# gorse-io/gorse

Hardware: AMD Instinct MI355X
Metric: BPR positive-samples/sec (whole job, N GPUs) (higher is better)
Workload: dtype f32; 1 GPU; S-ml1m 6040x3706x994169 per rank (C2), nFactors=64; factors_finite=True

## Files before the change

### gorse_amd/capi.py

```python
import ctypes as C
import os

import numpy as np

HERE = os.path.dirname(os.path.abspath(__file__))
LIB_PATH = os.environ.get("GORSE_HIP_LIB") or os.path.join(HERE, "lib", "libgorse_hip.so")

OK, ERR_INVALID, ERR_HIP, ERR_CANCELLED, ERR_NO_DEVICE, ERR_RANGE, ERR_NOMEM = 0, -1, -2, -3, -4, -5, -6
BPR_HOGWILD_ATOMIC, BPR_SEQUENTIAL, BPR_HOGWILD_RACY, BPR_HOGWILD_STORES = 0, 1, 2, 3
DTYPE_F32, DTYPE_BF16 = 0, 1
METRIC_NEG_DOT, METRIC_EUCLIDEAN, METRIC_COSINE, METRIC_EUCLIDEAN_BF16 = 0, 1, 2, 3
PROF_BPR_UPDATE, PROF_BPR_SAMPLE, PROF_ALS_SWEEP, PROF_ALS_GRAM, PROF_BPR_SORT, PROF_COMM = 0, 1, 2, 3, 4, 5
COMM_ID_BYTES = 128
OPT_SGD, OPT_ADAM = 0, 1
PROF_TOPK_SCORE, PROF_TOPK_RESCORE, PROF_TOPK_SWEEP, PROF_TOPK_SELECT, PROF_TOPK_HIST, PROF_TOPK_REPLAY = 0, 1, 2, 3, 4, 5

_f32p = C.POINTER(C.c_float)
_i32p = C.POINTER(C.c_int32)
_i64p = C.POINTER(C.c_int64)
_f64p = C.POINTER(C.c_double)
_vp = C.c_void_p

SIGNATURES = {
    "gorse_hip_abi_version": (C.c_int32, []),
# ... 115 lines not shown
    "gorse_hip_test_set_sparse_table": (None, [C.c_int32]),
    "gorse_hip_test_set_sparse_probe": (None, [C.c_int32]),
    "gorse_hip_test_set_sparse_sym": (None, [C.c_int32, C.c_int32, C.c_int32, C.c_int32]),
    "gorse_hip_test_set_sparse_front": (None, [C.c_int32]),
    "gorse_hip_test_sparse_sym_stats": (None, [C.c_void_p, C.POINTER(C.c_int64)]),
    "gorse_hip_test_set_sparse_tile": (None, [C.c_int32]),
    "gorse_hip_test_set_scan_literal": (None, [C.c_int32]),
    "gorse_hip_test_set_stream_priorities": (None, [C.c_int32]),
    "gorse_hip_test_set_sparse_split": (None, [C.c_int64]),
    "gorse_hip_test_set_sparse_heavy": (None, [C.c_int64]),
    "gorse_hip_test_set_sparse_atomic": (None, [C.c_int32]),
    "gorse_hip_test_set_als_path": (None, [C.c_int32]),
    "gorse_hip_test_set_als_plan": (None, [C.c_int32, C.c_int32]),
    "gorse_hip_test_set_bpr_chunk": (None, [C.c_int64]),
    "gorse_hip_test_bpr_prepare_chunk": (C.c_int32, [_vp, C.c_int64, C.c_uint64, C.c_uint64, C.c_int64, _i32p, _i32p, _i32p]),
    "gorse_hip_test_bpr_finish_capacities": (None, [_i32p, _i32p]),
    "gorse_hip_test_bpr_fail_count": (C.c_int32, [_vp, _i32p]),
    "gorse_hip_test_set_bpr_store_mode": (None, [C.c_int32]),
    "gorse_hip_test_set_prep_cu_stride": (None, [C.c_int32]),
    "gorse_hip_test_set_sgemm_valu": (None, [C.c_int32]),
    "gorse_hip_test_sgemm_last_ms": (C.c_double, []),
    "gorse_hip_test_set_bpr_cold_window": (None, [C.c_int64]),
    "gorse_hip_test_set_bpr_replica_unit": (None, [C.c_double]),
    "gorse_hip_test_set_bpr_fold_period": (None, [C.c_int32]),
    "gorse_hip_test_bpr_fold_stats": (C.c_int32, [_vp, _vp]),
    "gorse_hip_test_bpr_hot_state": (C.c_int32, [_vp, _vp, _vp, _vp]),
    "gorse_hip_test_set_recommend": (None, [C.c_int32, C.c_int32, C.c_int64]),
    "gorse_hip_test_set_fm_rank": (None, [C.c_int64, C.c_int32]),
    "gorse_hip_test_fm_rank_sort": (C.c_int32, [_vp, C.c_int64, _i64p, _f32p, _i32p]),
    "gorse_hip_test_set_fm_evaluate": (None, [C.c_int64, C.c_int32]),
# ... 161 lines not shown
    def bpr_sample_triplets(self, n, seed, epoch, sample_base=0):
        u = np.empty(n, np.int32)
        i = np.empty(n, np.int32)
        j = np.empty(n, np.int32)
        check(lib().gorse_bpr_sample_triplets(self.h, n, seed, epoch, sample_base, _p(u, _i32p), _p(i, _i32p),
                                              _p(j, _i32p)))
        return u, i, j

    def bpr_prepare_chunk(self, n, seed, epoch, sample_base=0):
        off = np.empty(self.U + 2, np.int32)
        si = np.empty(n, np.int32)
        sj = np.empty(n, np.int32)
        check(lib().gorse_hip_test_bpr_prepare_chunk(self.h, n, seed, epoch, sample_base, _p(off, _i32p), _p(si, _i32p),
                                                     _p(sj, _i32p)))
        return off, si, sj

    def bpr_fail_count(self):
        n = C.c_int32(0)
        check(lib().gorse_hip_test_bpr_fail_count(self.h, C.byref(n)))
        return n.value

    def bpr_apply_triplets(self, u, i, j, lr, reg, mode):
        u, i, j = _arr(u, np.int32), _arr(i, np.int32), _arr(j, np.int32)
        if not (u.size == i.size == j.size):
            raise GorseHipError(ERR_INVALID, "triplet arrays differ in length")
        check(lib().gorse_bpr_apply_triplets(self.h, _p(u, _i32p), _p(i, _i32p), _p(j, _i32p), u.size, lr, reg, mode))

    def als_epoch(self, weight, reg, cancel=None):
        cp = _p(cancel, _i32p) if cancel is not None else None
        check(lib().gorse_als_epoch(self.h, weight, reg, cp))
# ... 625 lines not shown
```

### gorse_amd/csrc/bpr.hip

```cpp
#include <algorithm>
#include <cstdlib>
#include <cstring>

#include "bpr_bins.hpp"
#include "mf_internal.hpp"
#include <utility>

using namespace gorse;

namespace {

int g_variant = 0;
constexpr int MODE_ATOMIC = GORSE_BPR_HOGWILD_ATOMIC;
constexpr int MODE_EXACT = GORSE_BPR_SEQUENTIAL;
constexpr int MODE_RACY = GORSE_BPR_HOGWILD_RACY;
constexpr int MODE_STORES = GORSE_BPR_HOGWILD_STORES;

__device__ __forceinline__ bool row_contains(const int32_t *__restrict__ row, int64_t n, int32_t x) {
    int64_t lo = 0, hi = n;
    while (lo < hi) {
        int64_t mid = (lo + hi) >> 1;
        if (row[mid] < x)
            lo = mid + 1;
        else
// ... 977 lines not shown
        su[pos] = us[s];
        si[pos] = is[s];
        sj[pos] = js[s];
    }
}

constexpr int kCold = -2;
constexpr int kSeriesFlush = 8;
#ifndef GORSE_BPR_SERIES_SKIP_GATHERS
#define GORSE_BPR_SERIES_SKIP_GATHERS 1
#endif

#ifndef GORSE_BPR_D8_PAIRS
#define GORSE_BPR_D8_PAIRS 1
#endif
template <int NC, bool NEG_STORE, bool D8 = false>
__global__ __launch_bounds__(kBlock) void bpr_update_user_kernel(float *P, float *Q, const int32_t *__restrict__ si,
                                                                 const int32_t *__restrict__ sj,
                                                                 const int32_t *__restrict__ off, int32_t U, int d,
                                                                 float lr, float reg, int exp_mode, double *loss,
                                                                 HotRows hot, int folders, int neg_replicas) {
    if ((int)blockIdx.x < folders) {
        run_folders<true>(hot, Q, folders);
        return;
    }
    auto continues = [](int i0, int j0, int i1, int j1) { return i0 == i1 && (i0 | j0 | j1) >= 0 && i0 != j0 && i0 != j1; };
    const int glane = threadIdx.x & (kGroup - 1);
    const int lane = D8 ? (glane & 7) : glane;
    constexpr int SUBS = D8 && GORSE_BPR_D8_PAIRS ? 2 : 1;
    const bool writer = !D8 || SUBS == 2 || glane < 8;
    auto mad = [](float x, float y, float z) { return D8 ? x * y + z : fmaf(x, y, z); };
    auto tree8 = [](float v) { return SUBS == 2 ? group_tree8_halves(v) : group_tree8(v); };
    const int gib = threadIdx.x / kGroup;
    const int64_t group = ((int64_t)((int)blockIdx.x - folders) * kGroupsPerBlock + gib) * SUBS + (SUBS == 2 ? glane >> 3 : 0);
    const int64_t ngroups = (int64_t)((int)gridDim.x - folders) * kGroupsPerBlock * SUBS;
    const float nreg = -reg;
    double my_loss = 0.0;
    const bool look_i = hot.n_hot > 0;
    const bool look_j = (hot.n_hot > 0 && neg_replicas) || NEG_STORE;
    const int32_t *slot_of = (look_i || look_j) ? hot.slot : si;
    int im1 = -1, jm1 = -1, im2 = -1, jm2 = -1;
    for (int64_t u = group; u < U; u += ngroups) {
        const int beg = off[u], end = off[u + 1];
        if (beg >= end) continue;
        float *pu = P + u * d;
        constexpr int G = 2, IA = 3;
        constexpr int GB = NEG_STORE ? 1 : G;
        float p[NC], ra[G][NC], rb[GB][NC];
        const int last = end - 1;
        auto at = [&](int s) { return s <= last ? s : last; };
// ... 137 lines not shown
int32_t exclusive_scan_i32(int32_t *data, int64_t m, int32_t *tmp, hipStream_t st) {
    const int64_t nt = ceil_div(m, kScanTile);
    if (nt <= 16) {
        scan_small_kernel<<<dim3(1), dim3(256), 0, st>>>(data, m);
        GORSE_HIP_CHECK(hipGetLastError());
        return GORSE_OK;
    }
    scan_tile_sums_kernel<<<dim3((unsigned)nt), dim3(256), 0, st>>>(data, m, tmp);
    scan_sums_kernel<<<dim3(1), dim3(256), 0, st>>>(tmp, nt);
    scan_apply_kernel<<<dim3((unsigned)nt), dim3(256), 0, st>>>(data, m, tmp);
    GORSE_HIP_CHECK(hipGetLastError());
    return GORSE_OK;
}


int32_t launch_user_sort(gorse_mf *h, const int32_t *trip, int32_t *sorted, int32_t *bucket, int32_t *rank, int64_t n, size_t cap,
                         hipStream_t st, bool ranked) {
    const int64_t m = h->U + 2;
    const int64_t blocks = std::min<int64_t>(ceil_div(n, 256), 256 * 8);
    if (!ranked) {
        GORSE_HIP_CHECK(hipMemsetAsync(bucket, 0, (size_t)m * sizeof(int32_t), st));
        if (g_variant & (1 << 29))
            bpr_rank_kernel<<<dim3(1), dim3(1), 0, st>>>(trip, n, (int32_t)h->U, bucket, rank);
        else
            bpr_rank_kernel<<<dim3((unsigned)blocks), dim3(256), 0, st>>>(trip, n, (int32_t)h->U, bucket, rank);
    }
    GORSE_TRY(exclusive_scan_i32(bucket, m, h->scan_tmp2.p, st));
    bpr_scatter_by_kernel<<<dim3((unsigned)blocks), dim3(256), 0, st>>>(trip, trip, trip + cap, trip + 2 * cap, n,
                                                                       (int32_t)h->U, bucket, rank, sorted,
                                                                       sorted + cap, sorted + 2 * cap);
    GORSE_HIP_CHECK(hipGetLastError());
    return GORSE_OK;
}
int32_t ensure_user_sort(gorse_mf *h) {
    const int64_t m = h->U + 2;
    const size_t mat = prep_matrix_words(h->U, (int64_t)h->trip_cap);
    if ((size_t)m <= h->ubucket[0].n && h->scan_tmp2.n >= (size_t)ceil_div(m, kScanTile) && h->urank[0].n >= 2 * h->trip_cap &&
        h->ubins.n >= (size_t)2 * kMaxBins && h->ubinmat.n >= mat)
        return GORSE_OK;
    GORSE_TRY(mf_sync_streams(h));
    if (h->ubins.n < (size_t)2 * kMaxBins) GORSE_TRY(h->ubins.alloc((size_t)2 * kMaxBins));
    if (h->ubinmat.n < mat) GORSE_TRY(h->ubinmat.alloc(mat));
    for (int b = 0; b < 2; b++) {
        GORSE_TRY(h->ubucket[b].alloc((size_t)m));
        GORSE_TRY(h->urank[b].alloc(2 * h->trip_cap));
    }
    if (h->scan_tmp2.n < (size_t)ceil_div(m, kScanTile)) GORSE_TRY(h->scan_tmp2.alloc((size_t)ceil_div(m, kScanTile)));
    return GORSE_OK;
}
bool user_runs_supported(const gorse_mf *h) {
    return (h->d == 8 || h->d == 16 || h->d == 32 || h->d == 64 || h->d == 128) && (h->U >= 4096 || (g_variant & 128));
}

constexpr int kDefaultStoreMode = 1;
int g_store_mode = kDefaultStoreMode;

HotRows make_hot(const gorse_mf *h) {
    return HotRows{h->hot_slot.p, h->hot_items.p, h->hot_meta.p, h->hot_rep.p, h->hot_done.p, 0, h->d, 0, g_fold_period};
}
int open_hot(gorse_mf *h, HotRows &hot) {
    hot.n_hot = h->n_hot;
    hot.set = (int)(h->hot_launches++ & 1);
    return kFolderBlocks;
}

int32_t launch_update_users(gorse_mf *h, const int32_t *sorted, const int32_t *bucket, size_t cap, float lr, float reg,
                            int exp_mode, double *loss, hipStream_t st, bool stores, hipEvent_t start = nullptr,
                            hipEvent_t stop = nullptr) {
    const int d = h->d;
    int64_t blocks = ceil_div(h->U, (int64_t)kGroupsPerBlock * (d == 8 && GORSE_BPR_D8_PAIRS ? 2 : 1));
    const int64_t capb = 256 * 16;
    if (blocks > capb) blocks = capb;
    HotRows hot = make_hot(h);
    const int folders = h->n_hot > 0 && !(g_variant & 32) ? open_hot(h, hot) : 0;
    blocks += folders;
    const int neg_rep = !(g_variant & (1 << 25)) && hot.n_hot > 0 && hot_neg_replicas(hot.n_hot, h->I) ? 1 : 0;
    dim3 grid((unsigned)blocks), block(kBlock);
    const bool neg_store = stores && h->n_cold > 0 && g_store_mode == 1;
#define LAUNCH2(NC, NEG_STORE)                                                                                         \
    hipExtLaunchKernelGGL((bpr_update_user_kernel<(NC == 0 ? 1 : NC), NEG_STORE, NC == 0>), grid, block, 0, st, start, stop, 0,     \
                          h->P.p, h->Q.p, sorted + cap, sorted + 2 * cap, bucket, (int32_t)h->U, d, lr, reg, exp_mode, loss, hot, \
                          folders, neg_rep)
#define LAUNCH(NC)                                                                                                     \
    do {                                                                                                               \
        if (neg_store)                                                                                                 \
            LAUNCH2(NC, true);                                                                                         \
        else                                                                                                           \
            LAUNCH2(NC, false);                                                                                        \
    } while (0)
    if (d == 8)
        LAUNCH(0);
    else if (d == 16)
        LAUNCH(1);
    else if (d == 32)
        LAUNCH(2);
    else if (d == 64)
        LAUNCH(4);
// ... 59 lines not shown
int32_t launch_sampler(gorse_mf *h, uint64_t seed, uint64_t epoch, int64_t base, int64_t n, int32_t *trip, size_t cap,
                       hipStream_t st, int32_t *bucket = nullptr, int32_t *rank = nullptr, hipEvent_t start = nullptr,
                       hipEvent_t stop = nullptr) {
    if (n <= 0) return GORSE_OK;
    int64_t blocks = std::min<int64_t>(ceil_div(n, 256), 256 * 8);
    if (bucket) GORSE_HIP_CHECK(hipMemsetAsync(bucket, 0, (size_t)(h->U + 2) * sizeof(int32_t), st));
    hipExtLaunchKernelGGL(bpr_sample_kernel, dim3((unsigned)blocks), dim3(256), 0, st, start, stop, 0, (int32_t)h->U, (int32_t)h->I,
                          h->uptr.p, h->uidx.p, h->uidx_sorted.p, seed, epoch, base, n, trip, trip + cap, trip + 2 * cap,
                          h->fail_count.p, bucket, rank);
    GORSE_HIP_CHECK(hipGetLastError());
    return GORSE_OK;
}

constexpr size_t kItemsBatchFrom = (size_t)8 << 20;
int32_t launch_prepare_users(gorse_mf *h, uint64_t seed, uint64_t epoch, int64_t base, int64_t n, int32_t *trip, int32_t *sorted,
                             int32_t *bucket, int32_t *rank, size_t cap, hipStream_t st) {
    if (n <= 0) return GORSE_OK;
    const int64_t m = h->U + 2;
    const int64_t blocks = std::min<int64_t>(ceil_div(n, 256), 256 * 8);
    const PrepBins pb = prep_bins(h->U, n);
    hipEvent_t ev_a = nullptr, ev_b = nullptr;
    auto launch_items = [&](const int2 *pairs) {
        h->prof.events(GORSE_PROF_BPR_SAMPLE, &ev_a, &ev_b);
        if (h->uidx.n > kItemsBatchFrom)
            hipExtLaunchKernelGGL(bpr_sample_items_batch_kernel, dim3((unsigned)blocks), dim3(256), 0, st, ev_a, ev_b, 0, (int32_t)h->U,
                                  (int32_t)h->I, h->uptr.p, h->uidx.p, h->uidx_sorted.p, seed, epoch, base, n, pairs, sorted + cap,
                                  sorted + 2 * cap, h->fail_count.p);
        else
            hipExtLaunchKernelGGL(bpr_sample_items_kernel, dim3((unsigned)blocks), dim3(256), 0, st, ev_a, ev_b, 0, (int32_t)h->U,
                                  (int32_t)h->I, h->uptr.p, h->uidx.p, h->uidx_sorted.p, seed, epoch, base, n, pairs, sorted + cap,
                                  sorted + 2 * cap, h->fail_count.p);
    };
    auto launch_group = [&]() {
        if (g_variant & (1 << 20)) return;
        h->prof.events(GORSE_PROF_BPR_SORT, &ev_a, &ev_b);
        hipExtLaunchKernelGGL(bpr_group_positives_kernel, dim3((unsigned)std::min<int64_t>(h->U, 256 * 16)), dim3(64), 0, st, ev_a, ev_b, 0,
                              (int32_t)h->U, bucket, sorted + cap, sorted + 2 * cap);
    };
    if (pb.ok && !(g_variant & (1 << 21))) {
        int32_t *key = trip;
        int2 *bp = reinterpret_cast<int2 *>(trip + cap), *pairs = reinterpret_cast<int2 *>(rank);
        int32_t *bin_count = h->ubins.p, *bin_start = h->ubins.p + kMaxBins, *H = h->ubinmat.p;
        const unsigned tiles = (unsigned)ceil_div(n, pb.tile);
        if ((size_t)tiles * pb.nbins > h->ubinmat.n) return fail(GORSE_ERR_INVALID, "tile x bin matrix smaller than %u x %d", tiles, pb.nbins);
        const bool finish = !(g_variant & (1 << 19)) && pb.shift <= kFinShift && n / pb.nbins <= kFinCap / 4 * 3 &&
                            h->uidx.n <= kItemsBatchFrom;
        h->prof.events(GORSE_PROF_BPR_SAMPLE, &ev_a, &ev_b);
        hipExtLaunchKernelGGL(bpr_bin_count_kernel, dim3(tiles), dim3(kBinThreads), 0, st, ev_a, ev_b, 0, (int32_t)h->U, h->uptr.p, seed,
                              epoch, base, n, pb.tile, pb.shift, pb.nbins, key, h->fail_count.p, H);
        h->prof.events(GORSE_PROF_BPR_SORT, &ev_a, &ev_b);
        hipExtLaunchKernelGGL(bpr_bin_offsets_kernel, dim3((unsigned)ceil_div(pb.nbins, 64)), dim3(kOffWaves * 64), 0, st, ev_a, nullptr, 0,
                              H, (int)tiles, pb.nbins, bin_count);
        hipExtLaunchKernelGGL(bpr_bin_scatter_kernel, dim3(tiles), dim3(kBinThreads), 0, st, nullptr, finish ? ev_b : nullptr, 0,
                              (int32_t)h->U, key, n, pb.tile, pb.shift, pb.nbins, bin_count, H, bin_start, bp);
        if (finish) {
            h->prof.events(GORSE_PROF_BPR_SAMPLE, &ev_a, &ev_b);
            hipExtLaunchKernelGGL(bpr_bin_finish_kernel, dim3((unsigned)pb.nbins), dim3(kFinThreads), 0, st, ev_a, ev_b, 0, (int32_t)h->U,
                                  (int32_t)h->I, pb.shift, bin_start, bp, h->uptr.p, h->uidx.p, h->uidx_sorted.p, seed, epoch, base, bucket,
                                  pairs, sorted + cap, sorted + 2 * cap, h->fail_count.p, (g_variant & (1 << 20)) ? 0 : 1);
            GORSE_HIP_CHECK(hipGetLastError());
            return GORSE_OK;
        }
        hipExtLaunchKernelGGL(bpr_bin_sort_kernel, dim3((unsigned)pb.nbins), dim3(256), 0, st, nullptr, ev_b, 0, (int32_t)h->U, pb.shift,
                              pb.nbins, bin_start, bp, bucket, pairs);
        launch_items(pairs);
        launch_group();
        GORSE_HIP_CHECK(hipGetLastError());
        return GORSE_OK;
    }
    int32_t *key = trip;
    int2 *pairs = reinterpret_cast<int2 *>(trip + cap);
    int tok = h->prof.begin(GORSE_PROF_BPR_SAMPLE, st);
    GORSE_HIP_CHECK(hipMemsetAsync(bucket, 0, (size_t)m * sizeof(int32_t), st));
    bpr_sample_user_kernel<<<dim3((unsigned)blocks), dim3(256), 0, st>>>((int32_t)h->U, h->uptr.p, seed, epoch, base, n, key,
                                                                         h->fail_count.p, bucket, rank);
    h->prof.end(tok, st);
    tok = h->prof.begin(GORSE_PROF_BPR_SORT, st);
    GORSE_TRY(exclusive_scan_i32(bucket, m, h->scan_tmp2.p, st));
    bpr_scatter_ids_kernel<<<dim3((unsigned)blocks), dim3(256), 0, st>>>(key, rank, bucket, n, (int32_t)h->U, pairs);
    h->prof.end(tok, st);
    launch_items(pairs);
    launch_group();
    GORSE_HIP_CHECK(hipGetLastError());
    return GORSE_OK;
}

int64_t g_chunk_override = 0;
int64_t chunk_capacity(const gorse_mf *h) {
    if (g_chunk_override > 0) return g_chunk_override;
    const int64_t lo = (int64_t)1 << 22, hi = (int64_t)1 << 27;
    return std::min(std::max(lo, 32 * h->U), hi);
}

int32_t ensure_trip(gorse_mf *h, int64_t want) {
    size_t cap = (size_t)std::min<int64_t>(std::max<int64_t>(want, 1), chunk_capacity(h));
    cap = (cap + 1) & ~(size_t)1;
    if (cap <= h->trip_cap) return GORSE_OK;
    GORSE_TRY(mf_sync_streams(h));
    for (int b = 0; b < 2; b++) GORSE_TRY(h->trip[b].alloc(cap * 3));
// ... 97 lines not shown
        if (uruns) GORSE_TRY(ensure_user_sort(h));
        int64_t c = 0;
        for (int64_t s0 = 0; s0 < n_samples; s0 += cap, c++) {
            const int b = (int)(h->chunk_seq & 1);
            h->chunk_seq++;
            const int64_t m = std::min(cap, n_samples - s0);
            if (cancel && *cancel) {
                GORSE_TRY(mf_sync_streams(h));
                return fail(GORSE_ERR_CANCELLED, "cancelled");
            }
            int32_t *tb = h->trip[b].p;
            const hipStream_t prep = (g_variant & (1 << 22)) ? h->stream : h->stream2;
            if (h->ev_consumed[b]) GORSE_HIP_CHECK(hipStreamWaitEvent(prep, h->ev_consumed[b], 0));
            const bool fused = uruns && !(g_variant & (1 << 29)) && !(g_variant & (1 << 27));
            const bool by_run = fused && !(g_variant & (1 << 26));
            if (by_run) {
                GORSE_TRY(launch_prepare_users(h, seed, epoch, base + s0, m, tb, h->sorted[b].p, h->ubucket[b].p, h->urank[b].p,
                                               (size_t)cap, prep));
            } else {
                int tok = fused ? h->prof.begin(GORSE_PROF_BPR_SAMPLE, prep) : -1;
                hipEvent_t sa = nullptr, sb = nullptr;
                if (!fused) h->prof.events(GORSE_PROF_BPR_SAMPLE, &sa, &sb);
                GORSE_TRY(launch_sampler(h, seed, epoch, base + s0, m, tb, (size_t)cap, prep, fused ? h->ubucket[b].p : nullptr,
                                         fused ? h->urank[b].p : nullptr, sa, sb));
                h->prof.end(tok, prep);
                if (fused) {
                    tok = h->prof.begin(GORSE_PROF_BPR_SORT, prep);
                    GORSE_TRY(launch_user_sort(h, tb, h->sorted[b].p, h->ubucket[b].p, h->urank[b].p, m, (size_t)cap, prep, true));
                    h->prof.end(tok, prep);
                }
            }
            GORSE_HIP_CHECK(hipEventRecord(h->ev_sampled[b], prep));
            GORSE_HIP_CHECK(hipStreamWaitEvent(h->stream, h->ev_sampled[b], 0));
            if (uruns && !fused) {
                const int tok = h->prof.begin(GORSE_PROF_BPR_SORT, h->stream);
                GORSE_TRY(launch_user_sort(h, tb, h->sorted[b].p, h->ubucket[b].p, h->urank[b].p, m, (size_t)cap, h->stream, false));
                h->prof.end(tok, h->stream);
            }
            hipEvent_t start = nullptr, stop = nullptr;
            h->prof.events(GORSE_PROF_BPR_UPDATE, &start, &stop);
            const bool last = s0 + cap >= n_samples;
            if (!start && c == 0) start = ep_begin;
            if (!stop) stop = last ? mf_epoch_end_event(h) : h->ev_chunk[(h->chunk_seq - 1) % gorse_mf::kChunkRing];
            if (uruns)
                GORSE_TRY(launch_update_users(h, h->sorted[b].p, h->ubucket[b].p, (size_t)cap, lr, reg, g_exp_mode_exact, d_loss, h->stream,
                                              mode == MODE_STORES, start, stop));
            else
                GORSE_TRY(launch_update(h, mode == MODE_STORES ? MODE_ATOMIC : mode, tb, tb + cap, tb + 2 * cap, nullptr, 0, m, lr, reg, 0, d_loss,
                                        h->stream, start, stop));
            h->ev_consumed[b] = stop;
            if (last) ep_end = stop;
            if (cancel && (c & 7) == 7) GORSE_TRY(mf_sync_streams(h));
        }
    }
    GORSE_TRY(mf_epoch_end(h, ep_end));
    h->ep_chain = true;
    if (sync || loss_out) {
        if (loss_out)
            GORSE_HIP_CHECK(hipMemcpyAsync(loss_out, h->loss.p, sizeof(double), hipMemcpyDeviceToHost, h->stream));
        GORSE_TRY(mf_sync_streams(h));
        GORSE_TRY(mf_epoch_harvest(h, true));
// ... 89 lines not shown
extern "C" int32_t gorse_hip_test_bpr_prepare_chunk(gorse_mf *h, int64_t n, uint64_t seed, uint64_t epoch, int64_t sample_base,
                                                    int32_t *off , int32_t *si , int32_t *sj ) {
    if (!h || !off || !si || !sj) return fail(GORSE_ERR_INVALID, "NULL argument");
    GORSE_TRY(h->use());
    GORSE_TRY(ensure_trip(h, n));
    if (n < 0 || n > (int64_t)h->trip_cap) return fail(GORSE_ERR_INVALID, "n outside one chunk (%zu samples)", h->trip_cap);
    if (!user_runs_supported(h)) return fail(GORSE_ERR_INVALID, "this handle does not run the user-run schedule");
    GORSE_TRY(ensure_user_sort(h));
    GORSE_TRY(mf_sync_streams(h));
    const size_t cap = h->trip_cap;
    GORSE_TRY(launch_prepare_users(h, seed, epoch, sample_base, n, h->trip[0].p, h->sorted[0].p, h->ubucket[0].p, h->urank[0].p, cap,
                                   h->stream));
    GORSE_HIP_CHECK(hipMemcpyAsync(off, h->ubucket[0].p, (size_t)(h->U + 2) * 4, hipMemcpyDeviceToHost, h->stream));
    GORSE_HIP_CHECK(hipMemcpyAsync(si, h->sorted[0].p + cap, (size_t)n * 4, hipMemcpyDeviceToHost, h->stream));
    GORSE_HIP_CHECK(hipMemcpyAsync(sj, h->sorted[0].p + 2 * cap, (size_t)n * 4, hipMemcpyDeviceToHost, h->stream));
    GORSE_HIP_CHECK(hipStreamSynchronize(h->stream));
    return GORSE_OK;
}

extern "C" int32_t gorse_bpr_apply_triplets(gorse_mf *h, const int32_t *u, const int32_t *i, const int32_t *j, int64_t n,
                                            float lr, float reg, int32_t mode) {
    if (!h) return fail(GORSE_ERR_INVALID, "handle is NULL");
    if (n < 0 || (n > 0 && (!u || !i || !j))) return fail(GORSE_ERR_INVALID, "bad arguments");
    GORSE_TRY(check_mode(mode));
    if (n == 0) return GORSE_OK;
    for (int64_t s = 0; s < n; s++)
        if (u[s] >= h->U || i[s] >= h->I || j[s] >= h->I)
            return fail(GORSE_ERR_RANGE, "triplet %lld (%d,%d,%d) out of range", (long long)s, u[s], i[s], j[s]);
    GORSE_TRY(h->use());
    GORSE_TRY(ensure_trip(h, n));
    GORSE_TRY(mf_sync_streams(h));
    const int64_t cap = (int64_t)h->trip_cap;
    for (int64_t s0 = 0; s0 < n; s0 += cap) {
        const int64_t m = std::min(cap, n - s0);
        int32_t *tb = h->trip[0].p;
        GORSE_HIP_CHECK(hipMemcpyAsync(tb, u + s0, (size_t)m * 4, hipMemcpyHostToDevice, h->stream));
        GORSE_HIP_CHECK(hipMemcpyAsync(tb + cap, i + s0, (size_t)m * 4, hipMemcpyHostToDevice, h->stream));
        GORSE_HIP_CHECK(hipMemcpyAsync(tb + 2 * cap, j + s0, (size_t)m * 4, hipMemcpyHostToDevice, h->stream));
        if (mode == MODE_EXACT) {
            GORSE_TRY(run_sequential(h, tb, tb + cap, tb + 2 * cap, u + s0, i + s0, j + s0, m, lr, reg, g_exp_mode_exact,
                                     nullptr, nullptr));
        } else if ((mode == MODE_ATOMIC || mode == MODE_STORES) && user_runs_enabled() && user_runs_supported(h)) {
            GORSE_TRY(ensure_user_sort(h));
            GORSE_TRY(launch_user_sort(h, tb, h->sorted[0].p, h->ubucket[0].p, h->urank[0].p, m, (size_t)cap, h->stream, false));
            GORSE_TRY(launch_update_users(h, h->sorted[0].p, h->ubucket[0].p, (size_t)cap, lr, reg, g_exp_mode_exact, nullptr,
                                          h->stream, mode == MODE_STORES));
            GORSE_HIP_CHECK(hipStreamSynchronize(h->stream));
        } else {
            GORSE_TRY(launch_update(h, mode == MODE_STORES ? MODE_ATOMIC : mode, tb, tb + cap, tb + 2 * cap, nullptr, 0, m, lr, reg, 0, nullptr, h->stream));
            GORSE_HIP_CHECK(hipStreamSynchronize(h->stream));
        }
    }
    return GORSE_OK;
}
```

### gorse_amd/csrc/mf_internal.hpp

```cpp
#pragma once
#include <vector>

#include "cf_device.hpp"

#include "hot_rows.hpp"

#define GORSE_HOT_DONE_STRIPES 32
#define GORSE_HOT_DONE_STRIDE 64
#define GORSE_HOT_DONE_WORDS (2 * GORSE_HOT_DONE_STRIPES * GORSE_HOT_DONE_STRIDE + GORSE_HOT_DONE_STRIDE)
#ifndef GORSE_HOT_REPLICAS
#define GORSE_HOT_REPLICAS 8
#endif

struct gorse_mf {
    int device = 0;
    int64_t U = 0, I = 0, nnz = 0;
    int64_t max_user_row = 0, max_item_row = 0;
    int d = 0;
    bool has_item_csr = false;
    hipStream_t stream = nullptr;
    hipStream_t stream2 = nullptr;
    hipEvent_t ev_sampled[2] = {nullptr, nullptr};
    hipEvent_t ev_consumed[2] = {nullptr, nullptr};
    static constexpr int kChunkRing = 4;
// ... 3 lines not shown
    bool ep_events = false;
    bool ep_begin_prev[kEpochRing] = {};
    mutable bool ep_chain = false;
    uint64_t ep_seq = 0, ep_done = 0;
    double ep_ms = 0.0;
    int64_t ep_timed = 0;
    int64_t ep_untimed = 0;
    gorse::DevBuf<float> P, Q, Qsync;
    gorse::DevBuf<int64_t> uptr, iptr;
    gorse::DevBuf<int32_t> uidx, uidx_sorted, iidx;
    gorse::DevBuf<int32_t> trip[2];
    size_t trip_cap = 0;
    gorse::DevBuf<int32_t> sorted[2];
    gorse::DevBuf<int32_t> ubucket[2];
    gorse::DevBuf<int32_t> urank[2];
    gorse::DevBuf<int32_t> scan_tmp2;
    gorse::DevBuf<int32_t> ubins;
    gorse::DevBuf<int32_t> ubinmat;
    int64_t chunk_seq = 0;
    gorse::DevBuf<int32_t> hot_slot, hot_items, hot_meta, hot_done;
    gorse::DevBuf<float> hot_rep;
    int n_hot = 0;
    int64_t hot_rows = 0;
    uint64_t hot_launches = 0;
    int64_t n_cold = 0;
    int64_t cold_window = 0;
    std::vector<int32_t> h_item_count;
    std::vector<int32_t> h_hot_slot;
    gorse::DevBuf<int32_t> order;
    gorse::DevBuf<double> loss;
// ... 53 lines not shown
```

Baseline: 2.368 billion samples/s.

## Precompute per-sample control words and add lean user-run update loop

Adds a kernel, run after the user sort, that precomputes a packed control word per sample. Each word holds the series-continue, flush, send, accumulate and gather flags plus the byte offset of the target row (including hot-replica redirection). A new lean update loop reads these words and software-pipelines the Q row loads two samples ahead, replacing the per-sample branchy logic in the user-run update kernel. This costs an extra kernel launch and an 8-byte-per-sample control buffer in memory traffic. It also adds an explicit vmcnt wait on every iteration, which may limit the benefit of the prefetching.

```diff
diff --git a/gorse_amd/capi.py b/gorse_amd/capi.py
--- a/gorse_amd/capi.py
+++ b/gorse_amd/capi.py
@@ -153,6 +153,9 @@
     "gorse_hip_test_set_als_plan": (None, [C.c_int32, C.c_int32]),
     "gorse_hip_test_set_bpr_chunk": (None, [C.c_int64]),
     "gorse_hip_test_bpr_prepare_chunk": (C.c_int32, [_vp, C.c_int64, C.c_uint64, C.c_uint64, C.c_int64, _i32p, _i32p, _i32p]),
+    "gorse_hip_test_bpr_prepare_chunk_control": (C.c_int32, [_vp, C.c_int64, C.c_uint64, C.c_uint64, C.c_int64, C.c_int32, _i32p, _i32p, _i32p,
+                                                 _i32p]),
+    "gorse_hip_test_bpr_sort_control": (C.c_int32, [_vp, _i32p, _i32p, _i32p, C.c_int64, C.c_int32, _i32p, _i32p, _i32p, _i32p]),
     "gorse_hip_test_bpr_finish_capacities": (None, [_i32p, _i32p]),
     "gorse_hip_test_bpr_fail_count": (C.c_int32, [_vp, _i32p]),
     "gorse_hip_test_set_bpr_store_mode": (None, [C.c_int32]),
@@ -344,6 +347,22 @@
         check(lib().gorse_hip_test_bpr_prepare_chunk(self.h, n, seed, epoch, sample_base, _p(off, _i32p), _p(si, _i32p),
                                                      _p(sj, _i32p)))
         return off, si, sj
+
+    def bpr_prepare_chunk_control(self, n, seed, epoch, sample_base=0, mode=BPR_HOGWILD_ATOMIC):
+        off = np.empty(self.U + 2, np.int32)
+        si, sj, ctl = np.empty(n, np.int32), np.empty(n, np.int32), np.empty((n, 2), np.int32)
+        check(lib().gorse_hip_test_bpr_prepare_chunk_control(self.h, n, seed, epoch, sample_base, mode, _p(off, _i32p), _p(si, _i32p),
+                                                             _p(sj, _i32p), _p(ctl, _i32p)))
+        return off, si, sj, ctl
+
+    def bpr_sort_control(self, u, i, j, mode=BPR_HOGWILD_ATOMIC):
+        u, i, j = _arr(u, np.int32), _arr(i, np.int32), _arr(j, np.int32)
+        n = u.size
+        off = np.empty(self.U + 2, np.int32)
+        si, sj, ctl = np.empty(n, np.int32), np.empty(n, np.int32), np.empty((n, 2), np.int32)
+        check(lib().gorse_hip_test_bpr_sort_control(self.h, _p(u, _i32p), _p(i, _i32p), _p(j, _i32p), n, mode, _p(off, _i32p),
+                                                    _p(si, _i32p), _p(sj, _i32p), _p(ctl, _i32p)))
+        return off, si, sj, ctl
 
     def bpr_fail_count(self):
         n = C.c_int32(0)
diff --git a/gorse_amd/csrc/bpr.hip b/gorse_amd/csrc/bpr.hip
--- a/gorse_amd/csrc/bpr.hip
+++ b/gorse_amd/csrc/bpr.hip
@@ -1015,17 +1015,177 @@
 #ifndef GORSE_BPR_D8_PAIRS
 #define GORSE_BPR_D8_PAIRS 1
 #endif
+__device__ __forceinline__ bool series_continues(int i0, int j0, int i1, int j1) {
+    return i0 == i1 && (i0 | j0 | j1) >= 0 && i0 != j0 && i0 != j1;
+}
+
+#ifndef GORSE_BPR_LEAN_LOOP
+#define GORSE_BPR_LEAN_LOOP 1
+#endif
+constexpr uint32_t kCtlValid = 1;
+constexpr uint32_t kCtlCont = 2;
+constexpr uint32_t kCtlMore = 4;
+constexpr uint32_t kCtlFlush = 8;
+constexpr uint32_t kCtlGather = 16;
+constexpr uint32_t kCtlRep = 0x80000000u, kCtlOffset = 0x7fffffc0u;
+constexpr uint32_t kCtlSend = 1;
+constexpr uint32_t kCtlAccum = 2;
+constexpr uint32_t kCtlGather2 = 4;
+
+__global__ __launch_bounds__(64) void bpr_run_control_kernel(int32_t U, const int32_t *__restrict__ off, const int32_t *__restrict__ si,
+                                                             const int32_t *__restrict__ sj, const int32_t *__restrict__ slot_of,
+                                                             int d, int32_t ngroups, int neg_replicas, int2 *__restrict__ ctl) {
+    const int lane = threadIdx.x;
+    const uint32_t rowb = (uint32_t)d * 4u;
+    auto cl = [](int x) { return x < 0 ? 0 : x; };
+    auto target = [&](const int32_t *slots, int it, int g) {
+        const int32_t code = slots && it >= 0 ? slots[it] : -1;
+        if (code >= 0) return (uint32_t)(hot_base(code) + (g & ((1 << hot_lg(code)) - 1))) * rowb | kCtlRep;
+        return (uint32_t)cl(it) * rowb;
+    };
+    for (int32_t u = blockIdx.x; u < U; u += gridDim.x) {
+        const int beg = off[u], end = off[u + 1];
+        const int g = u % ngroups;
+        int carry = 0;
+        for (int w = beg; w < end; w += 64) {
+            const int s = w + lane;
+            const bool in = s < end;
+            auto ld = [&](const int32_t *a, int t) { return t >= beg && t < end ? a[t] : -1; };
+            const int i = ld(si, s), j = ld(sj, s);
+            const bool cont = in && s > beg && series_continues(ld(si, s - 1), ld(sj, s - 1), i, j);
+            const bool more = in && s + 1 < end && series_continues(i, j, ld(si, s + 1), ld(sj, s + 1));
+            const bool cont2 = s + 2 < end && series_continues(ld(si, s + 1), ld(sj, s + 1), ld(si, s + 2), ld(sj, s + 2));
+            const uint64_t starts = ~__ballot(cont) & (lane == 63 ? ~0ull : (2ull << lane) - 1);
+            const int pos = starts ? lane - (63 - __clzll((long long)starts)) : carry + lane + 1;
+            carry = __shfl(pos, 63, 64);
+            if (!in) continue;
+            const bool flush = (pos & (kSeriesFlush - 1)) == kSeriesFlush - 1;
+            const bool gather = !GORSE_BPR_SERIES_SKIP_GATHERS || !cont;
+            const bool gather2 = s + 2 < end && (!GORSE_BPR_SERIES_SKIP_GATHERS || !cont2);
+            uint32_t x = target(slot_of, i, g), y = target(neg_replicas ? slot_of : nullptr, j, g);
+            x |= (j >= 0 ? kCtlValid : 0) | (cont ? kCtlCont : 0) | (more ? kCtlMore : 0) | (flush ? kCtlFlush : 0) | (gather ? kCtlGather : 0);
+            y |= (!more || flush ? kCtlSend : 0) | ((pos & (kSeriesFlush - 1)) != 0 ? kCtlAccum : 0) | (gather2 ? kCtlGather2 : 0);
+            ctl[s] = make_int2((int)x, (int)y);
+        }
+    }
+}
+
+constexpr int kLeanUnroll = 3;
+#ifndef GORSE_BPR_LEAN_WAIT
+#define GORSE_BPR_LEAN_WAIT 1
+#endif
+template <int NC>
+__device__ __forceinline__ void bpr_user_runs_lean(float *P, float *Q, float *rep, const int32_t *__restrict__ si,
+                                                   const int32_t *__restrict__ sj, const int2 *__restrict__ ctl,
+                                                   const int32_t *__restrict__ off, int32_t U, int d, float lr, float reg, int exp_mode,
+                                                   double *loss, int64_t group, int64_t ngroups, int lane) {
+    const float nreg = -reg;
+    double my_loss = 0.0;
+    const uint32_t rowb = (uint32_t)d * 4u, laneb = (uint32_t)lane * 4u;
+    auto cl = [](int x) { return x < 0 ? 0 : x; };
+    auto qrow = [&](int item) { return reinterpret_cast<const float *>(reinterpret_cast<const char *>(Q) + ((uint32_t)cl(item) * rowb + laneb)); };
+    auto word = [](const int32_t *a, uint32_t pos) { return *reinterpret_cast<const int32_t *>(reinterpret_cast<const char *>(a) + pos * 4u); };
+    auto cword = [&](uint32_t pos) { return *reinterpret_cast<const int2 *>(reinterpret_cast<const char *>(ctl) + pos * 8u); };
+    auto target = [&](uint32_t w) {
+        return reinterpret_cast<float *>(reinterpret_cast<char *>((int32_t)w < 0 ? rep : Q) + ((w & kCtlOffset) + laneb));
+    };
+    for (int64_t u = group; u < U; u += ngroups) {
+        const int beg = off[u], end = off[u + 1];
+        if (beg >= end) continue;
+        float *pu = P + u * d;
+        const int last = end - 1;
+        auto at = [&](int s) { return (uint32_t)(s <= last ? s : last); };
+        float p[NC], ra[2][NC], rb[2][NC], cur[NC], acc[NC];
+        int gi[2], gj[2];
+        int2 cw[2];
+#pragma unroll
+        for (int k = 0; k < 2; k++) cw[k] = cword(at(beg + k)), gi[k] = word(si, at(beg + 2 + k)), gj[k] = word(sj, at(beg + 2 + k));
+        {
+            const int i0 = word(si, at(beg)), j0 = word(sj, at(beg)), i1 = word(si, at(beg + 1)), j1 = word(sj, at(beg + 1));
+#pragma unroll
+            for (int c = 0; c < NC; c++) {
+                p[c] = load_row<MODE_ATOMIC>(pu + 16 * c + lane);
+                ra[0][c] = load_row<MODE_ATOMIC>(qrow(i0) + 16 * c);
+                ra[1][c] = load_row<MODE_ATOMIC>(qrow(i1) + 16 * c);
+                rb[0][c] = load_row<MODE_ATOMIC>(qrow(j0) + 16 * c);
+                rb[1][c] = load_row<MODE_ATOMIC>(qrow(j1) + 16 * c);
+            }
+        }
+        for (int s = beg; s < end;) {
+#pragma unroll
+            for (int k = 0; k < kLeanUnroll; k++, s++) {
+                const uint32_t w = (uint32_t)cw[0].x, w2 = (uint32_t)cw[0].y;
+                const int gin = word(si, at(s + 4)), gjn = word(sj, at(s + 4));
+                const int2 cwn = cword(at(s + 2));
+                float(&a)[NC] = ra[0];
+                float(&b)[NC] = rb[0];
+                float ran[NC], rbn[NC];
+#pragma unroll
+                for (int c = 0; c < NC; c++) ran[c] = 0.0f;
+                if (w2 & kCtlGather2) {
+#pragma unroll
+                    for (int c = 0; c < NC; c++) ran[c] = load_row<MODE_ATOMIC>(qrow(gi[0]) + 16 * c);
+                }
+#pragma unroll
+                for (int c = 0; c < NC; c++) rbn[c] = load_row<MODE_ATOMIC>(qrow(gj[0]) + 16 * c);
+                if (w & kCtlCont) {
+#pragma unroll
+                    for (int c = 0; c < NC; c++) a[c] = cur[c];
+                }
+                const bool valid = (w & kCtlValid) != 0 && s < end;
+                const float diff = dot512_regs<NC>(p, a) - dot512_regs<NC>(p, b);
+                const float ex = bpr_exp(-diff, exp_mode);
+                const float grad = ex / (1.0f + ex);
+                if (loss && lane == 0 && valid) my_loss += (double)log1pf(ex);
+                float t1[NC], t2[NC];
+#pragma unroll
+                for (int c = 0; c < NC; c++) {
+                    t1[c] = fmaf(a[c], nreg, p[c] * grad);
+                    t2[c] = fmaf(b[c], nreg, p[c] * (-grad));
+                    const float t3 = fmaf(p[c], nreg, (a[c] - b[c]) * grad);
+                    p[c] = valid ? fmaf(t3, lr, p[c]) : p[c];
+                }
+                if (valid) {
+#pragma unroll
+                    for (int c = 0; c < NC; c++) {
+                        acc[c] = (w2 & kCtlAccum) ? acc[c] + t1[c] * lr : t1[c] * lr;
+                        cur[c] = fmaf(t1[c], lr, a[c]);
+                    }
+                    if (w2 & kCtlSend) {
+                        float *qi = target(w);
+#pragma unroll
+                        for (int c = 0; c < NC; c++) __hip_atomic_fetch_add(qi + 16 * c, acc[c], __ATOMIC_RELAXED, __HIP_MEMORY_SCOPE_AGENT);
+                    }
+                    float *qj = target(w2);
+#pragma unroll
+                    for (int c = 0; c < NC; c++) __hip_atomic_fetch_add(qj + 16 * c, t2[c] * lr, __ATOMIC_RELAXED, __HIP_MEMORY_SCOPE_AGENT);
+                }
+                if (GORSE_BPR_LEAN_WAIT) asm volatile("s_waitcnt vmcnt(0)" ::: "memory");
+#pragma unroll
+                for (int c = 0; c < NC; c++) ra[0][c] = ra[1][c], ra[1][c] = ran[c], rb[0][c] = rb[1][c], rb[1][c] = rbn[c];
+                cw[0] = cw[1], cw[1] = cwn;
+                gi[0] = gi[1], gi[1] = gin, gj[0] = gj[1], gj[1] = gjn;
+            }
+        }
+#pragma unroll
+        for (int c = 0; c < NC; c++)
+            __hip_atomic_store(pu + 16 * c + lane, p[c], __ATOMIC_RELAXED, __HIP_MEMORY_SCOPE_AGENT);
+    }
+    if (loss && lane == 0 && my_loss != 0.0) atomicAdd(loss, my_loss);
+}
+
 template <int NC, bool NEG_STORE, bool D8 = false>
 __global__ __launch_bounds__(kBlock) void bpr_update_user_kernel(float *P, float *Q, const int32_t *__restrict__ si,
                                                                  const int32_t *__restrict__ sj,
                                                                  const int32_t *__restrict__ off, int32_t U, int d,
                                                                  float lr, float reg, int exp_mode, double *loss,
-                                                                 HotRows hot, int folders, int neg_replicas) {
+                                                                 HotRows hot, int folders, int neg_replicas,
+                                                                 const int2 *__restrict__ ctl) {
     if ((int)blockIdx.x < folders) {
         run_folders<true>(hot, Q, folders);
         return;
     }
-    auto continues = [](int i0, int j0, int i1, int j1) { return i0 == i1 && (i0 | j0 | j1) >= 0 && i0 != j0 && i0 != j1; };
+    auto continues = [](int i0, int j0, int i1, int j1) { return series_continues(i0, j0, i1, j1); };
     const int glane = threadIdx.x & (kGroup - 1);
     const int lane = D8 ? (glane & 7) : glane;
     constexpr int SUBS = D8 && GORSE_BPR_D8_PAIRS ? 2 : 1;
@@ -1035,6 +1195,13 @@
     const int gib = threadIdx.x / kGroup;
     const int64_t group = ((int64_t)((int)blockIdx.x - folders) * kGroupsPerBlock + gib) * SUBS + (SUBS == 2 ? glane >> 3 : 0);
     const int64_t ngroups = (int64_t)((int)gridDim.x - folders) * kGroupsPerBlock * SUBS;
+    if constexpr (GORSE_BPR_LEAN_LOOP && !NEG_STORE && !D8) {
+        if (ctl) {
+            bpr_user_runs_lean<NC>(P, Q, hot.rep, si, sj, ctl, off, U, d, lr, reg, exp_mode, loss, group, ngroups, glane);
+            if (folders > 0) worker_done<true>(hot);
+            return;
+        }
+    }
     const float nreg = -reg;
     double my_loss = 0.0;
     const bool look_i = hot.n_hot > 0;
@@ -1202,8 +1369,34 @@
 }
 
 
+int g_store_mode_value();
+int64_t user_run_blocks(const gorse_mf *h) {
+    const int64_t blocks = ceil_div(h->U, (int64_t)kGroupsPerBlock * (h->d == 8 && GORSE_BPR_D8_PAIRS ? 2 : 1));
+    return std::min<int64_t>(blocks, 256 * 16);
+}
+int64_t user_run_groups(const gorse_mf *h) { return user_run_blocks(h) * kGroupsPerBlock * (h->d == 8 && GORSE_BPR_D8_PAIRS ? 2 : 1); }
+bool user_runs_open_hot(const gorse_mf *h) { return h->n_hot > 0 && !(g_variant & 32); }
+bool user_runs_neg_replicas(const gorse_mf *h) {
+    return !(g_variant & (1 << 25)) && user_runs_open_hot(h) && hot_neg_replicas(h->n_hot, h->I);
+}
+bool lean_eligible(const gorse_mf *h, bool stores) {
+    if (!GORSE_BPR_LEAN_LOOP || (g_variant & (1 << 18))) return false;
+    if (h->d != 16 && h->d != 32 && h->d != 64 && h->d != 128) return false;
+    if (stores && h->n_cold > 0 && g_store_mode_value() == 1) return false;
+    return (h->I + h->hot_rows) * (int64_t)h->d * 4 < ((int64_t)1 << 31);
+}
+int32_t launch_run_control(gorse_mf *h, const int32_t *sorted, const int32_t *bucket, size_t cap, int32_t *ctl, hipStream_t st,
+                           hipEvent_t start = nullptr, hipEvent_t stop = nullptr) {
+    const int32_t *slots = user_runs_open_hot(h) ? h->hot_slot.p : nullptr;
+    hipExtLaunchKernelGGL(bpr_run_control_kernel, dim3((unsigned)std::min<int64_t>(h->U, 256 * 16)), dim3(64), 0, st, start, stop, 0,
+                          (int32_t)h->U, bucket, sorted + cap, sorted + 2 * cap, slots, h->d, (int32_t)user_run_groups(h),
+                          user_runs_neg_replicas(h) ? 1 : 0, reinterpret_cast<int2 *>(ctl));
+    GORSE_HIP_CHECK(hipGetLastError());
+    return GORSE_OK;
+}
+
 int32_t launch_user_sort(gorse_mf *h, const int32_t *trip, int32_t *sorted, int32_t *bucket, int32_t *rank, int64_t n, size_t cap,
-                         hipStream_t st, bool ranked) {
+                         hipStream_t st, bool ranked, int32_t *ctl = nullptr) {
     const int64_t m = h->U + 2;
     const int64_t blocks = std::min<int64_t>(ceil_div(n, 256), 256 * 8);
     if (!ranked) {
@@ -1218,13 +1411,14 @@
                                                                        (int32_t)h->U, bucket, rank, sorted,
                                                                        sorted + cap, sorted + 2 * cap);
     GORSE_HIP_CHECK(hipGetLastError());
+    if (ctl) GORSE_TRY(launch_run_control(h, sorted, bucket, cap, ctl, st));
     return GORSE_OK;
 }
 int32_t ensure_user_sort(gorse_mf *h) {
     const int64_t m = h->U + 2;
     const size_t mat = prep_matrix_words(h->U, (int64_t)h->trip_cap);
     if ((size_t)m <= h->ubucket[0].n && h->scan_tmp2.n >= (size_t)ceil_div(m, kScanTile) && h->urank[0].n >= 2 * h->trip_cap &&
-        h->ubins.n >= (size_t)2 * kMaxBins && h->ubinmat.n >= mat)
+        h->uctl[0].n >= 2 * h->trip_cap && h->ubins.n >= (size_t)2 * kMaxBins && h->ubinmat.n >= mat)
         return GORSE_OK;
     GORSE_TRY(mf_sync_streams(h));
     if (h->ubins.n < (size_t)2 * kMaxBins) GORSE_TRY(h->ubins.alloc((size_t)2 * kMaxBins));
@@ -1232,6 +1426,7 @@
     for (int b = 0; b < 2; b++) {
         GORSE_TRY(h->ubucket[b].alloc((size_t)m));
         GORSE_TRY(h->urank[b].alloc(2 * h->trip_cap));
+        GORSE_TRY(h->uctl[b].alloc(2 * h->trip_cap));
     }
     if (h->scan_tmp2.n < (size_t)ceil_div(m, kScanTile)) GORSE_TRY(h->scan_tmp2.alloc((size_t)ceil_div(m, kScanTile)));
     return GORSE_OK;
@@ -1242,6 +1437,7 @@
 
 constexpr int kDefaultStoreMode = 1;
 int g_store_mode = kDefaultStoreMode;
+int g_store_mode_value() { return g_store_mode; }
 
 HotRows make_hot(const gorse_mf *h) {
     return HotRows{h->hot_slot.p, h->hot_items.p, h->hot_meta.p, h->hot_rep.p, h->hot_done.p, 0, h->d, 0, g_fold_period};
@@ -1254,21 +1450,20 @@
 
 int32_t launch_update_users(gorse_mf *h, const int32_t *sorted, const int32_t *bucket, size_t cap, float lr, float reg,
                             int exp_mode, double *loss, hipStream_t st, bool stores, hipEvent_t start = nullptr,
-                            hipEvent_t stop = nullptr) {
+                            hipEvent_t stop = nullptr, const int32_t *ctl = nullptr) {
     const int d = h->d;
-    int64_t blocks = ceil_div(h->U, (int64_t)kGroupsPerBlock * (d == 8 && GORSE_BPR_D8_PAIRS ? 2 : 1));
-    const int64_t capb = 256 * 16;
-    if (blocks > capb) blocks = capb;
+    int64_t blocks = user_run_blocks(h);
     HotRows hot = make_hot(h);
-    const int folders = h->n_hot > 0 && !(g_variant & 32) ? open_hot(h, hot) : 0;
+    const int folders = user_runs_open_hot(h) ? open_hot(h, hot) : 0;
     blocks += folders;
-    const int neg_rep = !(g_variant & (1 << 25)) && hot.n_hot > 0 && hot_neg_replicas(hot.n_hot, h->I) ? 1 : 0;
+    const int neg_rep = user_runs_neg_replicas(h) ? 1 : 0;
+    if (ctl && !lean_eligible(h, stores)) return fail(GORSE_ERR_INVALID, "a control stream for a launch that cannot walk the lean loop");
     dim3 grid((unsigned)blocks), block(kBlock);
     const bool neg_store = stores && h->n_cold > 0 && g_store_mode == 1;
 #define LAUNCH2(NC, NEG_STORE)                                                                                         \
     hipExtLaunchKernelGGL((bpr_update_user_kernel<(NC == 0 ? 1 : NC), NEG_STORE, NC == 0>), grid, block, 0, st, start, stop, 0,     \
                           h->P.p, h->Q.p, sorted + cap, sorted + 2 * cap, bucket, (int32_t)h->U, d, lr, reg, exp_mode, loss, hot, \
-                          folders, neg_rep)
+                          folders, neg_rep, reinterpret_cast<const int2 *>(ctl))
 #define LAUNCH(NC)                                                                                                     \
     do {                                                                                                               \
         if (neg_store)                                                                                                 \
@@ -1358,7 +1553,7 @@
 
 constexpr size_t kItemsBatchFrom = (size_t)8 << 20;
 int32_t launch_prepare_users(gorse_mf *h, uint64_t seed, uint64_t epoch, int64_t base, int64_t n, int32_t *trip, int32_t *sorted,
-                             int32_t *bucket, int32_t *rank, size_t cap, hipStream_t st) {
+                             int32_t *bucket, int32_t *rank, size_t cap, hipStream_t st, int32_t *ctl = nullptr) {
     if (n <= 0) return GORSE_OK;
     const int64_t m = h->U + 2;
     const int64_t blocks = std::min<int64_t>(ceil_div(n, 256), 256 * 8);
@@ -1381,6 +1576,11 @@
         hipExtLaunchKernelGGL(bpr_group_positives_kernel, dim3((unsigned)std::min<int64_t>(h->U, 256 * 16)), dim3(64), 0, st, ev_a, ev_b, 0,
                               (int32_t)h->U, bucket, sorted + cap, sorted + 2 * cap);
     };
+    auto launch_control = [&]() -> int32_t {
+        if (!ctl) return GORSE_OK;
+        h->prof.events(GORSE_PROF_BPR_SORT, &ev_a, &ev_b);
+        return launch_run_control(h, sorted, bucket, cap, ctl, st, ev_a, ev_b);
+    };
     if (pb.ok && !(g_variant & (1 << 21))) {
         int32_t *key = trip;
         int2 *bp = reinterpret_cast<int2 *>(trip + cap), *pairs = reinterpret_cast<int2 *>(rank);
@@ -1399,10 +1599,11 @@
                               (int32_t)h->U, key, n, pb.tile, pb.shift, pb.nbins, bin_count, H, bin_start, bp);
         if (finish) {
             h->prof.events(GORSE_PROF_BPR_SAMPLE, &ev_a, &ev_b);
-            hipExtLaunchKernelGGL(bpr_bin_finish_kernel, dim3((unsigned)pb.nbins), dim3(kFinThreads), 0, st, ev_a, ev_b, 0, (int32_t)h->U,
-                                  (int32_t)h->I, pb.shift, bin_start, bp, h->uptr.p, h->uidx.p, h->uidx_sorted.p, seed, epoch, base, bucket,
-                                  pairs, sorted + cap, sorted + 2 * cap, h->fail_count.p, (g_variant & (1 << 20)) ? 0 : 1);
+            hipExtLaunchKernelGGL(bpr_bin_finish_kernel, dim3((unsigned)pb.nbins), dim3(kFinThreads), 0, st, ev_a, ctl ? nullptr : ev_b, 0,
+                                  (int32_t)h->U, (int32_t)h->I, pb.shift, bin_start, bp, h->uptr.p, h->uidx.p, h->uidx_sorted.p, seed, epoch, base,
+                                  bucket, pairs, sorted + cap, sorted + 2 * cap, h->fail_count.p, (g_variant & (1 << 20)) ? 0 : 1);
             GORSE_HIP_CHECK(hipGetLastError());
+            if (ctl) GORSE_TRY(launch_run_control(h, sorted, bucket, cap, ctl, st, nullptr, ev_b));
             return GORSE_OK;
         }
         hipExtLaunchKernelGGL(bpr_bin_sort_kernel, dim3((unsigned)pb.nbins), dim3(256), 0, st, nullptr, ev_b, 0, (int32_t)h->U, pb.shift,
@@ -1410,7 +1611,7 @@
         launch_items(pairs);
         launch_group();
         GORSE_HIP_CHECK(hipGetLastError());
-        return GORSE_OK;
+        return launch_control();
     }
     int32_t *key = trip;
     int2 *pairs = reinterpret_cast<int2 *>(trip + cap);
@@ -1426,7 +1627,7 @@
     launch_items(pairs);
     launch_group();
     GORSE_HIP_CHECK(hipGetLastError());
-    return GORSE_OK;
+    return launch_control();
 }
 
 int64_t g_chunk_override = 0;
@@ -1554,9 +1755,10 @@
             if (h->ev_consumed[b]) GORSE_HIP_CHECK(hipStreamWaitEvent(prep, h->ev_consumed[b], 0));
             const bool fused = uruns && !(g_variant & (1 << 29)) && !(g_variant & (1 << 27));
             const bool by_run = fused && !(g_variant & (1 << 26));
+            int32_t *ctl = uruns && lean_eligible(h, mode == MODE_STORES) ? h->uctl[b].p : nullptr;
             if (by_run) {
                 GORSE_TRY(launch_prepare_users(h, seed, epoch, base + s0, m, tb, h->sorted[b].p, h->ubucket[b].p, h->urank[b].p,
-                                               (size_t)cap, prep));
+                                               (size_t)cap, prep, ctl));
             } else {
                 int tok = fused ? h->prof.begin(GORSE_PROF_BPR_SAMPLE, prep) : -1;
                 hipEvent_t sa = nullptr, sb = nullptr;
@@ -1566,7 +1768,7 @@
                 h->prof.end(tok, prep);
                 if (fused) {
                     tok = h->prof.begin(GORSE_PROF_BPR_SORT, prep);
-                    GORSE_TRY(launch_user_sort(h, tb, h->sorted[b].p, h->ubucket[b].p, h->urank[b].p, m, (size_t)cap, prep, true));
+                    GORSE_TRY(launch_user_sort(h, tb, h->sorted[b].p, h->ubucket[b].p, h->urank[b].p, m, (size_t)cap, prep, true, ctl));
                     h->prof.end(tok, prep);
                 }
             }
@@ -1574,7 +1776,7 @@
             GORSE_HIP_CHECK(hipStreamWaitEvent(h->stream, h->ev_sampled[b], 0));
             if (uruns && !fused) {
                 const int tok = h->prof.begin(GORSE_PROF_BPR_SORT, h->stream);
-                GORSE_TRY(launch_user_sort(h, tb, h->sorted[b].p, h->ubucket[b].p, h->urank[b].p, m, (size_t)cap, h->stream, false));
+                GORSE_TRY(launch_user_sort(h, tb, h->sorted[b].p, h->ubucket[b].p, h->urank[b].p, m, (size_t)cap, h->stream, false, ctl));
                 h->prof.end(tok, h->stream);
             }
             hipEvent_t start = nullptr, stop = nullptr;
@@ -1584,7 +1786,7 @@
             if (!stop) stop = last ? mf_epoch_end_event(h) : h->ev_chunk[(h->chunk_seq - 1) % gorse_mf::kChunkRing];
             if (uruns)
                 GORSE_TRY(launch_update_users(h, h->sorted[b].p, h->ubucket[b].p, (size_t)cap, lr, reg, g_exp_mode_exact, d_loss, h->stream,
-                                              mode == MODE_STORES, start, stop));
+                                              mode == MODE_STORES, start, stop, ctl));
             else
                 GORSE_TRY(launch_update(h, mode == MODE_STORES ? MODE_ATOMIC : mode, tb, tb + cap, tb + 2 * cap, nullptr, 0, m, lr, reg, 0, d_loss,
                                         h->stream, start, stop));
@@ -1704,6 +1906,54 @@
     GORSE_HIP_CHECK(hipMemcpyAsync(off, h->ubucket[0].p, (size_t)(h->U + 2) * 4, hipMemcpyDeviceToHost, h->stream));
     GORSE_HIP_CHECK(hipMemcpyAsync(si, h->sorted[0].p + cap, (size_t)n * 4, hipMemcpyDeviceToHost, h->stream));
     GORSE_HIP_CHECK(hipMemcpyAsync(sj, h->sorted[0].p + 2 * cap, (size_t)n * 4, hipMemcpyDeviceToHost, h->stream));
+    GORSE_HIP_CHECK(hipStreamSynchronize(h->stream));
+    return GORSE_OK;
+}
+
+extern "C" int32_t gorse_hip_test_bpr_prepare_chunk_control(gorse_mf *h, int64_t n, uint64_t seed, uint64_t epoch, int64_t sample_base,
+                                                            int32_t mode, int32_t *off , int32_t *si , int32_t *sj ,
+                                                            int32_t *ctl ) {
+    if (!h || !off || !si || !sj || !ctl) return fail(GORSE_ERR_INVALID, "NULL argument");
+    GORSE_TRY(h->use());
+    GORSE_TRY(ensure_trip(h, n));
+    if (n < 0 || n > (int64_t)h->trip_cap) return fail(GORSE_ERR_INVALID, "n outside one chunk (%zu samples)", h->trip_cap);
+    if (!user_runs_supported(h)) return fail(GORSE_ERR_INVALID, "this handle does not run the user-run schedule");
+    if (!lean_eligible(h, mode == MODE_STORES)) return fail(GORSE_ERR_INVALID, "this handle's update launch takes no control stream");
+    GORSE_TRY(ensure_user_sort(h));
+    GORSE_TRY(mf_sync_streams(h));
+    const size_t cap = h->trip_cap;
+    GORSE_TRY(launch_prepare_users(h, seed, epoch, sample_base, n, h->trip[0].p, h->sorted[0].p, h->ubucket[0].p, h->urank[0].p, cap,
+                                   h->stream, h->uctl[0].p));
+    GORSE_HIP_CHECK(hipMemcpyAsync(off, h->ubucket[0].p, (size_t)(h->U + 2) * 4, hipMemcpyDeviceToHost, h->stream));
+    GORSE_HIP_CHECK(hipMemcpyAsync(si, h->sorted[0].p + cap, (size_t)n * 4, hipMemcpyDeviceToHost, h->stream));
+    GORSE_HIP_CHECK(hipMemcpyAsync(sj, h->sorted[0].p + 2 * cap, (size_t)n * 4, hipMemcpyDeviceToHost, h->stream));
+    GORSE_HIP_CHECK(hipMemcpyAsync(ctl, h->uctl[0].p, (size_t)n * 8, hipMemcpyDeviceToHost, h->stream));
+    GORSE_HIP_CHECK(hipStreamSynchronize(h->stream));
+    return GORSE_OK;
+}
+extern "C" int32_t gorse_hip_test_bpr_sort_control(gorse_mf *h, const int32_t *u, const int32_t *i, const int32_t *j, int64_t n, int32_t mode,
+                                                   int32_t *off , int32_t *si , int32_t *sj , int32_t *ctl ) {
+    if (!h || !u || !i || !j || !off || !si || !sj || !ctl) return fail(GORSE_ERR_INVALID, "NULL argument");
+    for (int64_t s = 0; s < n; s++)
+        if (u[s] >= h->U || i[s] >= h->I || j[s] >= h->I)
+            return fail(GORSE_ERR_RANGE, "triplet %lld (%d,%d,%d) out of range", (long long)s, u[s], i[s], j[s]);
+    GORSE_TRY(h->use());
+    GORSE_TRY(ensure_trip(h, n));
+    if (n <= 0 || n > (int64_t)h->trip_cap) return fail(GORSE_ERR_INVALID, "n outside one chunk (%zu samples)", h->trip_cap);
+    if (!user_runs_supported(h)) return fail(GORSE_ERR_INVALID, "this handle does not run the user-run schedule");
+    if (!lean_eligible(h, mode == MODE_STORES)) return fail(GORSE_ERR_INVALID, "this handle's update launch takes no control stream");
+    GORSE_TRY(ensure_user_sort(h));
+    GORSE_TRY(mf_sync_streams(h));
+    const size_t cap = h->trip_cap;
+    int32_t *tb = h->trip[0].p;
+    GORSE_HIP_CHECK(hipMemcpyAsync(tb, u, (size_t)n * 4, hipMemcpyHostToDevice, h->stream));
+    GORSE_HIP_CHECK(hipMemcpyAsync(tb + cap, i, (size_t)n * 4, hipMemcpyHostToDevice, h->stream));
+    GORSE_HIP_CHECK(hipMemcpyAsync(tb + 2 * cap, j, (size_t)n * 4, hipMemcpyHostToDevice, h->stream));
+    GORSE_TRY(launch_user_sort(h, tb, h->sorted[0].p, h->ubucket[0].p, h->urank[0].p, n, cap, h->stream, false, h->uctl[0].p));
+    GORSE_HIP_CHECK(hipMemcpyAsync(off, h->ubucket[0].p, (size_t)(h->U + 2) * 4, hipMemcpyDeviceToHost, h->stream));
+    GORSE_HIP_CHECK(hipMemcpyAsync(si, h->sorted[0].p + cap, (size_t)n * 4, hipMemcpyDeviceToHost, h->stream));
+    GORSE_HIP_CHECK(hipMemcpyAsync(sj, h->sorted[0].p + 2 * cap, (size_t)n * 4, hipMemcpyDeviceToHost, h->stream));
+    GORSE_HIP_CHECK(hipMemcpyAsync(ctl, h->uctl[0].p, (size_t)n * 8, hipMemcpyDeviceToHost, h->stream));
     GORSE_HIP_CHECK(hipStreamSynchronize(h->stream));
     return GORSE_OK;
 }
@@ -1732,9 +1982,10 @@
                                      nullptr, nullptr));
         } else if ((mode == MODE_ATOMIC || mode == MODE_STORES) && user_runs_enabled() && user_runs_supported(h)) {
             GORSE_TRY(ensure_user_sort(h));
-            GORSE_TRY(launch_user_sort(h, tb, h->sorted[0].p, h->ubucket[0].p, h->urank[0].p, m, (size_t)cap, h->stream, false));
+            int32_t *ctl = lean_eligible(h, mode == MODE_STORES) ? h->uctl[0].p : nullptr;
+            GORSE_TRY(launch_user_sort(h, tb, h->sorted[0].p, h->ubucket[0].p, h->urank[0].p, m, (size_t)cap, h->stream, false, ctl));
             GORSE_TRY(launch_update_users(h, h->sorted[0].p, h->ubucket[0].p, (size_t)cap, lr, reg, g_exp_mode_exact, nullptr,
-                                          h->stream, mode == MODE_STORES));
+                                          h->stream, mode == MODE_STORES, nullptr, nullptr, ctl));
             GORSE_HIP_CHECK(hipStreamSynchronize(h->stream));
         } else {
             GORSE_TRY(launch_update(h, mode == MODE_STORES ? MODE_ATOMIC : mode, tb, tb + cap, tb + 2 * cap, nullptr, 0, m, lr, reg, 0, nullptr, h->stream));
diff --git a/gorse_amd/csrc/mf_internal.hpp b/gorse_amd/csrc/mf_internal.hpp
--- a/gorse_amd/csrc/mf_internal.hpp
+++ b/gorse_amd/csrc/mf_internal.hpp
@@ -41,6 +41,7 @@
     gorse::DevBuf<int32_t> sorted[2];
     gorse::DevBuf<int32_t> ubucket[2];
     gorse::DevBuf<int32_t> urank[2];
+    gorse::DevBuf<int32_t> uctl[2];
     gorse::DevBuf<int32_t> scan_tmp2;
     gorse::DevBuf<int32_t> ubins;
     gorse::DevBuf<int32_t> ubinmat;
```

New measurement: 2.321 billion samples/s. 0.98x the previous value.
